# ShengkaiWu/IoU-aware-single-stage-object-detector

Hardware: AMD Instinct MI355X
Metric: images/sec at 1333x800, IoU-aware RetinaNet R-50-FPN (higher is better)
Workload: dtype fp32; 1 GPU; IoU-aware RetinaNet R-50-FPN fp32, batch 8 per GPU, 3x800x1344 (1333x800 padded to /32), random-init weights, whole inference path incl. NMS, device-to-host copy and bbox2result (the reference's simple_test: per-class arrays on the host; batch i's host part runs under batch i+1's device part, the last one inside the timed region); global_batch=8, parallelism=dp1, dets_per_image=100

## Files before the change

include/iouaware.h:

```cpp
#ifndef IOUAWARE_H
#define IOUAWARE_H

#include <stddef.h>
#include <stdint.h>

#ifdef __cplusplus
extern "C" {
#endif

#define IA_MAX_LEVELS 8
#define IA_MAX_ANCHORS 16
#define IA_MAX_NMS_PRE 4096
#define IA_MAX_CANDIDATES 8192
#define IA_MAX_PER_IMG 1024

#define IA_F32 0
#define IA_BF16 1
#define IA_F16 2
#define IA_F64 3

#define IA_LAYOUT_NCHW 0
#define IA_LAYOUT_NHWC 1

#define IA_CLS_SIGMOID 0
// ... 83 lines not shown
                       void *workspace, size_t workspace_bytes, float *dets, int32_t *labels,
                       int32_t *rows, int32_t *num, void *stream);

size_t ia_multiclass_nms_lazy_workspace_bytes(int batch, int R, int C);
int ia_multiclass_nms_lazy(const float *boxes, const float *scores_t, const float *best_score,
                           int batch, int R, int C, float score_thr, float iou_thr,
                           int max_per_img, int candidates, void *workspace,
                           size_t workspace_bytes, float *dets, int32_t *labels, int32_t *rows,
                           int32_t *num, void *stream);

int ia_decode_stage(const ia_head_geom *g, const ia_level_ptrs *p, int batch, int dtype,
                    const float *img_hw, const float *scale_factor, int rescale, void *workspace,
                    size_t workspace_bytes, void *stream);

int ia_get_bboxes_workspace_layout(const ia_head_geom *g, int batch, size_t offsets[8]);

size_t ia_nms_workspace_bytes(int n);
int ia_nms(const float *dets, int n, float iou_thr, int32_t *keep, int32_t *count, void *workspace,
           size_t workspace_bytes, void *stream);

size_t ia_nms_f64_workspace_bytes(int n);
int ia_nms_f64(const double *dets, int n, float iou_thr, int32_t *keep, int32_t *count,
               void *workspace, size_t workspace_bytes, void *stream);

int ia_soft_nms(const float *dets, int n, float iou_thr, int method, float sigma, float min_score,
                float *out_dets, int32_t *out_inds, int32_t *count, void *stream);

typedef struct {
    const uint8_t *src;
    int32_t src_h, src_w, dst_h, dst_w, flip;
} ia_image_desc;
int ia_image_transform(const ia_image_desc *imgs, int batch, const float *mean, const float *std,
                       int to_rgb, int pad_h, int pad_w, int channels_last, float *out,
                       void *stream);

typedef struct {
    int32_t num_levels, batch;
    int32_t H[IA_MAX_LEVELS], W[IA_MAX_LEVELS];
} ia_wino_geom;
typedef struct {
    int32_t c0, n;
    int32_t dst_channels, dst_offset;
    float *dst[IA_MAX_LEVELS];
} ia_wino_seg;
int ia_wino_tiles(const ia_wino_geom *g, int32_t *tiles);
int ia_wino_input_transform(const ia_wino_geom *g, const float *const *x, int channels, int groups,
                            const float *pre_scale, const float *pre_shift, int pre_relu, float *V,
                            void *stream);
int ia_wino_output_transform(const ia_wino_geom *g, const float *M, int channels, int groups,
                             const float *bias, int relu, int nseg, const ia_wino_seg *segs,
                             void *stream);
int ia_wino_mid_transform(const ia_wino_geom *g, const float *M, int channels, int groups_m,
                          const float *bias, int relu, float *V, int groups_v, void *stream);

int ia_wino_grad_output_transform(const ia_wino_geom *g, const float *const *dy, int channels,
                                  float *dM, void *stream);

#define IA_COLSUM_MAX_STRIPS 512
size_t ia_relu_bwd_bias_grad_workspace_bytes(int64_t rows, int n);
int ia_wino_weight_transform(const float *w, int n_in, int n_out, int64_t stride_in,
                             int64_t stride_out, int64_t stride_ky, int64_t stride_kx, int flip,
                             const double *G, float *U, void *stream);
int ia_wino_weight_grad(const float *dU, int n_in, int n_out, const double *G, float *dW,
                        int64_t stride_in, int64_t stride_out, int64_t stride_ky, int64_t stride_kx,
                        void *stream);
int ia_bn_fold_fwd(const float *w, const float *gamma, const float *beta, const float *mean,
                   const float *inv_std, int cout, int K, float *w_out, float *b_out, void *stream);
int ia_bn_fold_bwd(const float *dw_folded, const float *db_folded, const float *w, const float *gamma,
                   const float *mean, const float *inv_std, int cout, int K, float *dw,
                   float *dgamma, float *dbeta, void *stream);
int ia_relu_bwd_bias_grad(const float *dy, const float *y, int64_t rows, int n, float *g, float *db,
                          void *workspace, size_t workspace_bytes, void *stream);

int ia_linear_bias_act(const float *A, const float *W, const float *bias, const float *residual,
                       float *D, int64_t rows, int k, int n, int relu, void *workspace,
                       size_t workspace_bytes, void *stream);
int ia_linear_bias_act_bf16(const void *A, const void *W, const float *bias, const void *residual,
                            void *D, int64_t rows, int k, int n, int relu, void *workspace,
                            size_t workspace_bytes, void *stream);
int ia_batched_gemm(const float *A, const float *W, float *D, int batch, int64_t rows, int k, int n,
                    void *workspace, size_t workspace_bytes, void *stream);
int ia_batched_gemm_stream(const float *A, const float *W, float *D, int batch, int64_t rows, int k,
                           int n, void *stream);

size_t ia_im2col3x3_bytes(int B, int H, int W, int C, int stride, int dtype);
int ia_im2col3x3_nhwc(const void *x, void *col, int B, int H, int W, int C, int stride, int dtype,
                      void *stream);
int ia_conv1x1_strided(const void *x, const void *W_kn, const float *bias, const void *residual,
                       void *D, int B, int H, int W, int k, int n, int stride, int relu, int dtype,
                       void *workspace, size_t workspace_bytes, void *stream);
int ia_col2im3x3_nhwc(const void *dcol, void *dx, int B, int H, int W, int C, int stride, int dtype,
                      void *stream);

int ia_gemm_tuning(int mode);

int ia_gemm_table_add(int64_t m, int64_t n, int64_t k, int flags, int batch, int dtype,
                      int solution_index);
int ia_gemm_table_clear(void);
int ia_gemm_table_dump(int64_t *rows7, int capacity);
int ia_gemm_table_stats(int64_t *hits_misses_stale);
int ia_gemm_library_version(void);

int ia_linear_bias_act_wt(const float *A, const float *W_nk, const float *bias,
                          const float *residual, float *D, int64_t rows, int k, int n, int relu,
                          void *workspace, size_t workspace_bytes, void *stream);
int ia_gemm_tn(const float *G, const float *X, float *D, int batch, int64_t rows, int n, int k,
               void *workspace, size_t workspace_bytes, void *stream);


int ia_focal_loss_fwd(const void *cls, int dtype, const int64_t *labels,
                      const float *label_weights, int B, int A, int C, int HW, float gamma,
                      float alpha, double *loss_sum, void *stream);
int ia_focal_loss_bwd(const void *cls, int dtype, const int64_t *labels,
                      const float *label_weights, int B, int A, int C, int HW, float gamma,
                      float alpha, float gscale, const float *gscale_dev, float *grad_cls,
                      void *stream);

int ia_smooth_l1_fwd(const void *pred, int dtype, const float *target, const float *weight,
                     int B, int A, int HW, float beta, double *loss_sum, void *stream);
int ia_smooth_l1_bwd(const void *pred, int dtype, const float *target, const float *weight,
                     int B, int A, int HW, float beta, float gscale, const float *gscale_dev,
                     float *grad_pred, void *stream);

int ia_focal_loss_balanced_fwd(const void *cls, int dtype, const int64_t *labels,
                               const float *label_weights, const float *anchor_iou, int B, int A,
                               int C, int HW, float gamma, float alpha, float eta,
                               double *loss_sums3, void *stream);
int ia_focal_loss_balanced_bwd(const void *cls, int dtype, const int64_t *labels,
                               const float *label_weights, const float *anchor_iou, int B, int A,
                               int C, int HW, float gamma, float alpha, float eta,
                               const float *normalizer_dev, float gscale, const float *gscale_dev,
                               float *grad_cls, void *stream);
int ia_smooth_l1_balanced_fwd(const void *pred, int dtype, const float *target,
                              const float *weight, const float *anchor_iou, int B, int A, int HW,
                              float beta, float delta, double *loss_sum, void *stream);
int ia_smooth_l1_balanced_bwd(const void *pred, int dtype, const float *target,
                              const float *weight, const float *anchor_iou, int B, int A, int HW,
                              float beta, float delta, float gscale, const float *gscale_dev,
                              float *grad_pred, void *stream);

int ia_iou_bce_fwd(const ia_head_geom *g, int level, const void *bbox_pred, const void *iou_pred,
                   int dtype, const float *bbox_targets, const float *bbox_weights, int B,
                   float *iou_target, double *loss_sum, void *stream);
int ia_iou_bce_bwd(const ia_head_geom *g, int level, const void *bbox_pred, const void *iou_pred,
                   int dtype, const float *bbox_targets, const float *bbox_weights, int B,
                   float gscale, const float *gscale_dev, float *grad_iou_pred,
                   float *grad_bbox_pred, void *stream);

int ia_anchor_targets(const ia_head_geom *g, const float *gt_boxes, const int64_t *gt_labels,
                      const int32_t *num_gt, int batch, int gmax, const int32_t *valid_hw,
                      float pos_iou_thr, float neg_iou_thr, float min_pos_iou, float pos_weight,
                      uint32_t *gt_max_scratch, int64_t *labels, float *label_weights,
                      float *bbox_targets, float *bbox_weights, int32_t *counts, void *stream);

#define IA_MAX_TARGET_BATCH 16
int ia_anchor_targets_ptrs(const ia_head_geom *g, const float *const *gt_boxes,
                           const int64_t *const *gt_labels, const int32_t *num_gt, int batch,
                           const int32_t *valid_hw, float pos_iou_thr, float neg_iou_thr,
                           float min_pos_iou, float pos_weight, uint32_t *gt_max_scratch,
                           int64_t *labels, float *label_weights, float *bbox_targets,
                           float *bbox_weights, int32_t *counts, void *stream);

typedef struct ia_head_targets {
    const int64_t *labels[IA_MAX_LEVELS];
    const float *label_weights[IA_MAX_LEVELS];
    const float *bbox_targets[IA_MAX_LEVELS];
// ... 252 lines not shown
```

iou-aware-single-stage-object-detector_amd/csrc/build.py:

```python
import os
import subprocess
import sys

HERE = os.path.dirname(os.path.abspath(__file__))
SOURCES = ['capi.hip', 'decode.hip', 'select.hip', 'nms.hip', 'loss.hip', 'elementwise.hip', 'assign.hip',
           'softnms.hip', 'preproc.hip', 'wino.hip', 'gemm.hip', 'lazynms.hip', 'headloss.hip', 'gconv.hip',
           'trainops.hip', 'bignms.hip', 'conv3x3_bf16.hip', 'conv3x3_bf16_bwd.hip', 'conv1x1_stream.hip', 'im2col.hip', 'nms64.hip', 'stem.hip',
           'groupnorm.hip', 'pointdecode.hip', 'pointloss.hip', 'gconv_bf16.hip']
HEADERS = ['ia_math.hpp', 'ia_block.hpp', 'ia_internal.hpp', 'ia_loss.hpp', 'ia_headloss.hpp', 'ia_rowmax_dev.hpp', 'ia_gather_dev.hpp', 'ia_nms.hpp', 'ia_conv3.hpp', 'ia_wino.hpp', '../../include/iouaware.h']
OUT = os.path.join(HERE, 'libiouaware_hip.so')
FLAGS = ['--offload-arch=gfx950', '-O3', '-std=c++17', '-fPIC', '-ffp-contract=off',
         '-fhip-fp32-correctly-rounded-divide-sqrt', '-fno-gpu-rdc',
         '-Wall', '-Wno-unused-function']


def _hipcc():
    for c in (os.environ.get('HIPCC'), '/opt/rocm/bin/hipcc', 'hipcc'):
        if c and (os.path.isabs(c) and os.path.exists(c) or not os.path.isabs(c)):
            return c
    return 'hipcc'


def needs_build():
    if not os.path.exists(OUT):
        return True
    t = os.path.getmtime(OUT)
    deps = [os.path.join(HERE, f) for f in SOURCES + HEADERS] + [os.path.abspath(__file__)]
    return any(os.path.getmtime(d) > t for d in deps)


def build(force=False, verbose=False):
    if not force and not needs_build():
        return OUT
    objs = []
    procs = []
    for src in SOURCES:
        obj = os.path.join(HERE, src.replace('.hip', '.o'))
        cmd = [_hipcc()] + FLAGS + ['-c', os.path.join(HERE, src), '-o', obj]
        if verbose:
            print(' '.join(cmd))
        procs.append((src, subprocess.Popen(cmd, stdout=subprocess.PIPE, stderr=subprocess.STDOUT)))
        objs.append(obj)
    for src, pr in procs:
        out, _ = pr.communicate()
        if pr.returncode != 0:
            raise RuntimeError('hipcc failed on %s:\n%s' % (src, out.decode()))
        if verbose and out:
            print(out.decode())
    cmd = [_hipcc(), '--offload-arch=gfx950', '-shared', '-fPIC', '-o', OUT] + objs + [
        '-L/opt/rocm/lib', '-lhipblaslt', '-Wl,-rpath,/opt/rocm/lib']
    subprocess.run(cmd, check=True)
    return OUT


if __name__ == '__main__':
    print(build(force='--force' in sys.argv, verbose=True))
```

iou-aware-single-stage-object-detector_amd/csrc/ia_wino.hpp:

```cpp
#pragma once
#include "ia_internal.hpp"

namespace ia {

struct WinoLevels {
    int32_t L, B;
    int32_t H[IA_MAX_LEVELS], W[IA_MAX_LEVELS], tx[IA_MAX_LEVELS], tpi[IA_MAX_LEVELS];
    int32_t tile_off[IA_MAX_LEVELS + 1];
};

static inline int make_wino_levels(const ia_wino_geom *g, WinoLevels &w)
{
    if (!g || g->num_levels < 1 || g->num_levels > IA_MAX_LEVELS || g->batch < 1) return IA_E_ARG;
    w.L = g->num_levels; w.B = g->batch;
    w.tile_off[0] = 0;
    for (int l = 0; l < IA_MAX_LEVELS; ++l) {
        const bool on = l < g->num_levels;
        if (on && (g->H[l] < 1 || g->W[l] < 1)) return IA_E_ARG;
        w.H[l] = on ? g->H[l] : 0; w.W[l] = on ? g->W[l] : 0;
        w.tx[l] = (w.W[l] + 3) / 4;
        w.tpi[l] = ((w.H[l] + 3) / 4) * w.tx[l];
        const int64_t n = (int64_t)w.tile_off[l] + (int64_t)g->batch * w.tpi[l];
        if (n > 2147483647LL) return IA_E_ARG;
        w.tile_off[l + 1] = (int32_t)n;
    }
    return 0;
}

struct TileRef { int l, b, y0, x0; };

__device__ __forceinline__ int xcd_tile(int bid, int T)
{
    const int per = (T + 7) / 8;
    return (bid & 7) * per + (bid >> 3);
}

__device__ __forceinline__ TileRef locate_tile(const WinoLevels &w, int t, int *Hout = nullptr,
                                               int *Wout = nullptr)
{
    TileRef r;
    int l = 0;
#pragma unroll
    for (int i = 1; i < IA_MAX_LEVELS; ++i) l += (i < w.L && t >= w.tile_off[i]) ? 1 : 0;
    int off = w.tile_off[0], tpi = w.tpi[0], tx = w.tx[0], H = w.H[0], W = w.W[0];
#pragma unroll
    for (int i = 1; i < IA_MAX_LEVELS; ++i) {
        const bool m = l == i;
        off = m ? w.tile_off[i] : off; tpi = m ? w.tpi[i] : tpi; tx = m ? w.tx[i] : tx;
        H = m ? w.H[i] : H; W = m ? w.W[i] : W;
    }
    if (Hout) *Hout = H;
    if (Wout) *Wout = W;
    const int q = t - off;
    r.l = l; r.b = q / tpi;
    const int i = q - r.b * tpi;
    const int ty = i / tx;
    r.y0 = 4 * ty; r.x0 = 4 * (i - ty * tx);
    return r;
}

template <typename P>
__device__ __forceinline__ P opaque(P v)
{
    asm volatile("" : "+s"(v));
    return v;
}
template <bool UNIFORM, typename P>
__device__ __forceinline__ P level_ptr(P const (&tab)[IA_MAX_LEVELS], int l)
{
    if (UNIFORM) return tab[l];
    const char *base = reinterpret_cast<const char *>(tab[0]);
    int64_t d = 0;
#pragma unroll
    for (int i = 1; i < IA_MAX_LEVELS; ++i) {
        const int64_t di = opaque((int64_t)(reinterpret_cast<const char *>(tab[i]) - base));
        d = (l == i) ? di : d;
    }
    return reinterpret_cast<P>(const_cast<char *>(base + d));
}


constexpr int kMaxSeg = 4;

struct WinoSeg {
    int32_t c0, n, Cdst, coff;
    float *dst[IA_MAX_LEVELS];
};

}
```

iou-aware-single-stage-object-detector_amd/csrc/wino.hip:

```cpp
#include <string.h>
#include "ia_internal.hpp"
#include "ia_wino.hpp"

namespace ia {

typedef float f32x4_t __attribute__((ext_vector_type(4)));
__device__ __forceinline__ float4 load_nt(const float *p)
{
    const f32x4_t q = __builtin_nontemporal_load(reinterpret_cast<const f32x4_t *>(p));
    return make_float4(q.x, q.y, q.z, q.w);
}
__device__ __forceinline__ void store_nt(float *p, const float4 &v)
{
    f32x4_t q; q.x = v.x; q.y = v.y; q.z = v.z; q.w = v.w;
    __builtin_nontemporal_store(q, reinterpret_cast<f32x4_t *>(p));
}
__device__ __forceinline__ float4 f4(float v) { return make_float4(v, v, v, v); }
__device__ __forceinline__ float4 operator+(const float4 &a, const float4 &b) { return make_float4(a.x + b.x, a.y + b.y, a.z + b.z, a.w + b.w); }
__device__ __forceinline__ float4 operator-(const float4 &a, const float4 &b) { return make_float4(a.x - b.x, a.y - b.y, a.z - b.z, a.w - b.w); }
__device__ __forceinline__ float4 operator*(float s, const float4 &a) { return make_float4(s * a.x, s * a.y, s * a.z, s * a.w); }

__device__ __forceinline__ void bt6(const float4 (&d)[6], float4 (&o)[6])
{
    o[0] = (4.0f * d[0] - 5.0f * d[2]) + d[4];
    o[1] = (d[3] + d[4]) - 4.0f * (d[1] + d[2]);
    o[2] = 4.0f * (d[1] - d[2]) + (d[4] - d[3]);
    o[3] = 2.0f * (d[3] - d[1]) + (d[4] - d[2]);
    o[4] = 2.0f * (d[1] - d[3]) + (d[4] - d[2]);
    o[5] = (4.0f * d[1] - 5.0f * d[3]) + d[5];
}

__device__ __forceinline__ void at6(const float4 (&m)[6], float4 (&o)[4])
{
    const float4 s12 = m[1] + m[2], d12 = m[1] - m[2], s34 = m[3] + m[4], d34 = m[3] - m[4];
    o[0] = (m[0] + s12) + s34;
    o[1] = d12 + 2.0f * d34;
    o[2] = s12 + 4.0f * s34;
    o[3] = (d12 + 8.0f * d34) + m[5];
}

struct WinoInArgs {
    WinoLevels lv;
    const float *x[IA_MAX_LEVELS];
    float *V;
    const float *pre_scale, *pre_shift;
    int32_t Ctot, Cg, T, pre_relu, tpw;
};

struct LaneMap { int t, c; bool on; };
template <bool PACKED>
__device__ __forceinline__ LaneMap lane_map(int Ctot, int T, int tpw)
{
    LaneMap m;
    const int lane = threadIdx.x;
    if (PACKED) {
        const int q = Ctot >> 2;
        const int sub = lane / q;
        const int tw = xcd_tile(blockIdx.x, (T + tpw - 1) / tpw) * tpw + sub;
        m.t = tw; m.c = (lane - sub * q) * 4;
        m.on = (sub < tpw) && (tw < T);
    } else {
        m.t = __builtin_amdgcn_readfirstlane(xcd_tile(blockIdx.x, T));
        m.c = (blockIdx.y * 64 + lane) * 4;
        m.on = (m.c < Ctot) && (m.t < T);
    }
    return m;
}
static int tiles_per_wave(int channels)
{
    const int q = channels / 4;
    return (q < 64) ? (64 / q) : 1;
}

template <bool PACKED>
__global__ void __launch_bounds__(64) k_wino_in(WinoInArgs a)
{
    const LaneMap lm = lane_map<PACKED>(a.Ctot, a.T, a.tpw);
    if (!lm.on) return;
    const int t = lm.t, c = lm.c;
    int H, W;
    const TileRef r = locate_tile(a.lv, t, &H, &W);
    const float *x = level_ptr<!PACKED>(a.x, r.l) + (size_t)r.b * H * W * a.Ctot + c;
    const bool pre = a.pre_shift != nullptr;
    float4 ps = f4(1.0f), pb = f4(0.0f);
    if (pre) {
        if (a.pre_scale) ps = *reinterpret_cast<const float4 *>(a.pre_scale + c);
        pb = *reinterpret_cast<const float4 *>(a.pre_shift + c);
    }
    float4 d[6][6];
#pragma unroll
    for (int i = 0; i < 6; ++i) {
        const int y = r.y0 - 1 + i;
        const int yc = (y >= 0 && y < H) ? y : 0;
#pragma unroll
        for (int j = 0; j < 6; ++j) {
            const int xx = r.x0 - 1 + j;
            const int xc = (xx >= 0 && xx < W) ? xx : 0;
            d[i][j] = *reinterpret_cast<const float4 *>(x + ((size_t)yc * W + xc) * a.Ctot);
        }
    }
    if (pre) {
        const bool relu = a.pre_relu != 0;
#pragma unroll
        for (int i = 0; i < 6; ++i)
#pragma unroll
            for (int j = 0; j < 6; ++j) {
                float4 v = d[i][j];
                v = make_float4(v.x * ps.x + pb.x, v.y * ps.y + pb.y, v.z * ps.z + pb.z, v.w * ps.w + pb.w);
                const float4 z = make_float4(v.x > 0.f ? v.x : 0.f, v.y > 0.f ? v.y : 0.f,
                                             v.z > 0.f ? v.z : 0.f, v.w > 0.f ? v.w : 0.f);
                d[i][j] = relu ? z : v;
            }
    }
#pragma unroll
    for (int i = 0; i < 6; ++i) {
        const int y = r.y0 - 1 + i;
        const bool yin = (y >= 0) && (y < H);
#pragma unroll
        for (int j = 0; j < 6; ++j) {
            const int xx = r.x0 - 1 + j;
            const bool in = yin && (xx >= 0) && (xx < W);
// ... 416 lines not shown
```

iou-aware-single-stage-object-detector_amd/iouaware/_lib.py:

```python
import ctypes as C
import os

IA_MAX_LEVELS = 8
IA_MAX_ANCHORS = 16
IA_MAX_NMS_PRE = 4096
IA_MAX_CANDIDATES = 8192
IA_MAX_PER_IMG = 1024
IA_F32, IA_BF16, IA_F16, IA_F64 = 0, 1, 2, 3
IA_LAYOUT_NCHW, IA_LAYOUT_NHWC = 0, 1
IA_CLS_SIGMOID, IA_CLS_SOFTMAX = 0, 1
IA_CLS_SIGMOID_NOIOU, IA_CLS_SOFTMAX_NOIOU = 2, 3
IA_LOSS_SLOTS = 64
IA_MAX_TARGET_BATCH = 16
IA_GN_CHUNK = 256

_CSRC = os.path.join(os.path.dirname(os.path.abspath(__file__)), '..', 'csrc')
SO_PATH = os.path.abspath(os.path.join(_CSRC, 'libiouaware_hip.so'))


class HeadGeom(C.Structure):
    _fields_ = [('num_levels', C.c_int32), ('num_anchors', C.c_int32),
                ('num_classes', C.c_int32), ('nms_pre', C.c_int32),
                ('H', C.c_int32 * IA_MAX_LEVELS), ('W', C.c_int32 * IA_MAX_LEVELS),
                ('stride', C.c_int32 * IA_MAX_LEVELS),
# ... 49 lines not shown


class ImageDesc(C.Structure):
    _fields_ = [('src', C.c_void_p), ('src_h', C.c_int32), ('src_w', C.c_int32),
                ('dst_h', C.c_int32), ('dst_w', C.c_int32), ('flip', C.c_int32)]


class WinoGeom(C.Structure):
    _fields_ = [('num_levels', C.c_int32), ('batch', C.c_int32),
                ('H', C.c_int32 * IA_MAX_LEVELS), ('W', C.c_int32 * IA_MAX_LEVELS)]


class Conv3x3Desc(C.Structure):
    _fields_ = [('num_levels', C.c_int32), ('batch', C.c_int32), ('groups', C.c_int32),
                ('cin', C.c_int32), ('cout', C.c_int32), ('x_stride', C.c_int32), ('y_stride', C.c_int32),
                ('H', C.c_int32 * IA_MAX_LEVELS), ('W', C.c_int32 * IA_MAX_LEVELS),
                ('x', (C.c_void_p * IA_MAX_LEVELS) * 2), ('y', (C.c_void_p * IA_MAX_LEVELS) * 2)]


class WinoSeg(C.Structure):
    _fields_ = [('c0', C.c_int32), ('n', C.c_int32), ('dst_channels', C.c_int32),
                ('dst_offset', C.c_int32), ('dst', C.c_void_p * IA_MAX_LEVELS)]


_vp, _i, _f, _sz, _i64 = C.c_void_p, C.c_int, C.c_float, C.c_size_t, C.c_int64
_G, _P = C.POINTER(HeadGeom), C.POINTER(LevelPtrs)
_PG, _WG = C.POINTER(PointHeadGeom), C.POINTER(WinoGeom)
_PP, _PT, _PC = C.POINTER(PointLevelPtrs), C.POINTER(PointTargets), C.POINTER(PointLossCfg)

SIGNATURES = {
    'ia_version': (C.c_char_p, []),
    'ia_geom_sizes': (_i, [_G, C.POINTER(C.c_int32), C.POINTER(C.c_int32), C.POINTER(C.c_int32)]),
    'ia_decode_fuse_rowmax': (_i, [_G, _P, _i, _i, _vp, _vp]),
    'ia_select_topk_workspace_bytes': (_sz, [_G, _i]),
    'ia_select_topk': (_i, [_G, _vp, _i, _vp, _vp, _sz, _vp]),
    'ia_decode_fuse_rowmax_grouped': (_i, [_G, _P, _i, _i, _vp, _vp, _sz, _vp]),
    'ia_select_topk_grouped': (_i, [_G, _vp, _i, _vp, _vp, _sz, _vp]),
    'ia_decode_stage': (_i, [_G, _P, _i, _i, _vp, _vp, _i, _vp, _sz, _vp]),
    'ia_get_bboxes_status_offset': (_sz, [_G, _i]),
    'ia_debug_fused_spin_limit': (_i, [_i64]),
    'ia_profile_stage_events': (_i, [_vp, _vp]),
    'ia_gather_decode': (_i, [_G, _P, _i, _i, _vp, _vp, _vp, _i, _vp, _vp, _vp, _vp]),
    'ia_multiclass_nms_workspace_bytes': (_sz, [_i, _i, _i]),
    'ia_multiclass_nms': (_i, [_vp, _vp, _vp, _i, _i, _i, _f, _f, _i, _vp, _sz, _vp, _vp, _vp,
                               _vp, _vp, _vp, _vp]),
    'ia_multiclass_soft_nms_workspace_bytes': (_sz, [_i, _i, _i]),
    'ia_multiclass_soft_nms': (_i, [_vp, _vp, _i, _i, _i, _f, _f, _i, _f, _f, _i, _vp, _sz, _vp, _vp,
                                    _vp, _vp, _vp, _vp, _vp]),
    'ia_soft_nms': (_i, [_vp, _i, _f, _i, _f, _f, _vp, _vp, _vp, _vp]),
    'ia_get_bboxes_workspace_bytes': (_sz, [_G, _i]),
    'ia_get_bboxes': (_i, [_G, _P, _i, _i, _vp, _vp, _i, _f, _f, _i, _vp, _sz, _vp, _vp, _vp,
                           _vp, _vp]),
    'ia_multiclass_nms_lazy_workspace_bytes': (_sz, [_i, _i, _i]),
    'ia_multiclass_nms_lazy': (_i, [_vp, _vp, _vp, _i, _i, _i, _f, _f, _i, _i, _vp, _sz, _vp, _vp, _vp,
                                    _vp, _vp]),
    'ia_get_bboxes_lazy': (_i, [_G, _P, _i, _i, _vp, _vp, _i, _f, _f, _i, _i, _vp, _sz, _vp, _vp, _vp,
                                _vp, _vp]),
    'ia_get_bboxes_workspace_layout': (_i, [_G, _i, C.POINTER(_sz * 8)]),
    'ia_nms_workspace_bytes': (_sz, [_i]),
    'ia_nms': (_i, [_vp, _i, _f, _vp, _vp, _vp, _sz, _vp]),
    'ia_nms_f64_workspace_bytes': (_sz, [_i]),
    'ia_nms_f64': (_i, [_vp, _i, _f, _vp, _vp, _vp, _sz, _vp]),
    'ia_image_transform': (_i, [C.POINTER(ImageDesc), _i, C.POINTER(C.c_float), C.POINTER(C.c_float),
                                _i, _i, _i, _i, _vp, _vp]),
    'ia_wino_tiles': (_i, [C.POINTER(WinoGeom), C.POINTER(C.c_int32)]),
    'ia_wino_input_transform': (_i, [C.POINTER(WinoGeom), C.POINTER(C.c_void_p), _i, _i, _vp, _vp, _i,
                                     _vp, _vp]),
    'ia_wino_grad_output_transform': (_i, [C.POINTER(WinoGeom), C.POINTER(C.c_void_p), _i, _vp, _vp]),
    'ia_wino_weight_transform': (_i, [_vp, _i, _i, C.c_int64, C.c_int64, C.c_int64, C.c_int64, _i,
                                      C.POINTER(C.c_double), _vp, _vp]),
    'ia_wino_weight_grad': (_i, [_vp, _i, _i, C.POINTER(C.c_double), _vp, C.c_int64, C.c_int64,
                                 C.c_int64, C.c_int64, _vp]),
    'ia_bn_fold_fwd': (_i, [_vp, _vp, _vp, _vp, _vp, _i, _i, _vp, _vp, _vp]),
    'ia_bn_fold_bwd': (_i, [_vp, _vp, _vp, _vp, _vp, _vp, _i, _i, _vp, _vp, _vp, _vp]),
    'ia_relu_bwd_bias_grad_workspace_bytes': (C.c_size_t, [C.c_int64, _i]),
    'ia_relu_bwd_bias_grad': (_i, [_vp, _vp, C.c_int64, _i, _vp, _vp, _vp, C.c_size_t, _vp]),
    'ia_wino_output_transform': (_i, [C.POINTER(WinoGeom), _vp, _i, _i, _vp, _i, _i,
                                      C.POINTER(WinoSeg), _vp]),
    'ia_wino_mid_transform': (_i, [C.POINTER(WinoGeom), _vp, _i, _i, _vp, _i, _vp, _i, _vp]),
    'ia_linear_bias_act': (_i, [_vp, _vp, _vp, _vp, _vp, _i64, _i, _i, _i, _vp, _sz, _vp]),
    'ia_linear_bias_act_bf16': (_i, [_vp, _vp, _vp, _vp, _vp, _i64, _i, _i, _i, _vp, _sz, _vp]),
    'ia_batched_gemm': (_i, [_vp, _vp, _vp, _i, _i64, _i, _i, _vp, _sz, _vp]),
    'ia_batched_gemm_stream': (_i, [_vp, _vp, _vp, _i, _i64, _i, _i, _vp]),
    'ia_linear_bias_act_wt': (_i, [_vp, _vp, _vp, _vp, _vp, _i64, _i, _i, _i, _vp, _sz, _vp]),
    'ia_gemm_tuning': (_i, [_i]),
    'ia_im2col3x3_bytes': (_sz, [_i, _i, _i, _i, _i, _i]),
    'ia_im2col3x3_nhwc': (_i, [_vp, _vp, _i, _i, _i, _i, _i, _i, _vp]),
    'ia_col2im3x3_nhwc': (_i, [_vp, _vp, _i, _i, _i, _i, _i, _i, _vp]),
    'ia_conv1x1_strided': (_i, [_vp, _vp, _vp, _vp, _vp, _i, _i, _i, _i, _i, _i, _i, _i, _vp, _sz, _vp]),
    'ia_gemm_table_add': (_i, [_i64, _i64, _i64, _i, _i, _i, _i]),
    'ia_gemm_table_clear': (_i, []),
    'ia_gemm_table_dump': (_i, [_vp, _i]),
    'ia_gemm_table_stats': (_i, [_vp]),
    'ia_gemm_library_version': (_i, []),
    'ia_gemm_tn': (_i, [_vp, _vp, _vp, _i, _i64, _i, _i, _vp, _sz, _vp]),
    'ia_focal_loss_fwd': (_i, [_vp, _i, _vp, _vp, _i, _i, _i, _i, _f, _f, _vp, _vp]),
    'ia_focal_loss_bwd': (_i, [_vp, _i, _vp, _vp, _i, _i, _i, _i, _f, _f, _f, _vp, _vp, _vp]),
    'ia_smooth_l1_fwd': (_i, [_vp, _i, _vp, _vp, _i, _i, _i, _f, _vp, _vp]),
    'ia_smooth_l1_bwd': (_i, [_vp, _i, _vp, _vp, _i, _i, _i, _f, _f, _vp, _vp, _vp]),
    'ia_focal_loss_balanced_fwd': (_i, [_vp, _i, _vp, _vp, _vp, _i, _i, _i, _i, _f, _f, _f, _vp, _vp]),
    'ia_focal_loss_balanced_bwd': (_i, [_vp, _i, _vp, _vp, _vp, _i, _i, _i, _i, _f, _f, _f, _vp, _f,
                                        _vp, _vp, _vp]),
    'ia_smooth_l1_balanced_fwd': (_i, [_vp, _i, _vp, _vp, _vp, _i, _i, _i, _f, _f, _vp, _vp]),
    'ia_smooth_l1_balanced_bwd': (_i, [_vp, _i, _vp, _vp, _vp, _i, _i, _i, _f, _f, _f, _vp, _vp,
                                       _vp]),
    'ia_iou_bce_fwd': (_i, [_G, _i, _vp, _vp, _i, _vp, _vp, _i, _vp, _vp, _vp]),
    'ia_iou_bce_bwd': (_i, [_G, _i, _vp, _vp, _i, _vp, _vp, _i, _f, _vp, _vp, _vp, _vp]),
    'ia_anchor_targets': (_i, [_G, _vp, _vp, _vp, _i, _i, _vp, _f, _f, _f, _f, _vp, _vp, _vp, _vp,
                               _vp, _vp, _vp]),
    'ia_anchor_targets_ptrs': (_i, [_G, C.POINTER(C.c_void_p), C.POINTER(C.c_void_p),
                                    C.POINTER(C.c_int32), _i, C.POINTER(C.c_int32), _f, _f, _f, _f,
                                    _vp, _vp, _vp, _vp, _vp, _vp, _vp]),
    'ia_head_loss_workspace_bytes': (_sz, [_G, _i]),
    'ia_head_loss_fwd': (_i, [_G, _P, _i, _i, C.POINTER(HeadTargets), C.POINTER(HeadLossCfg), _vp,
                              _sz, _vp, _vp]),
    'ia_head_loss_bwd': (_i, [_G, _P, _i, _i, C.POINTER(HeadTargets), C.POINTER(HeadLossCfg), _vp,
                              _vp, _vp, _P, _vp]),
    'ia_head_loss_fwd_nhwc': (_i, [_G, _P, C.POINTER(LevelPixStrides), _i, C.POINTER(HeadTargets),
                                   C.POINTER(HeadLossCfg), _vp, _sz, _vp, _vp]),
    'ia_head_loss_bwd_nhwc': (_i, [_G, _P, C.POINTER(LevelPixStrides), _i, C.POINTER(HeadTargets),
                                   C.POINTER(HeadLossCfg), _vp, _vp, _P, C.POINTER(LevelPixStrides),
                                   _vp]),
    'ia_grouped_conv3x3_pack': (_i, [_vp, _vp, _i, _i, _vp]),
    'ia_grouped_conv3x3_nhwc': (_i, [_vp, _vp, _vp, _vp, _i, _i, _i, _i, _i, _i, _i, _vp]),
    'ia_grouped_conv3x3_packed_bytes_bf16': (C.c_size_t, [_i, _i]),
    'ia_grouped_conv3x3_pack_bf16': (_i, [_vp, _vp, _i, _i, _vp]),
    'ia_grouped_conv3x3_bf16_nhwc': (_i, [_vp, _vp, _vp, _vp, _i, _i, _i, _i, _i, _i, _i, _vp]),
    'ia_sigmoid_focal_loss_fwd': (_i, [_vp, _vp, _i, _i, _f, _f, _vp, _vp]),
    'ia_sigmoid_focal_loss_bwd': (_i, [_vp, _vp, _vp, _i, _i, _f, _f, _vp, _vp]),
    'ia_sigmoid_focal_loss_fwd_dt': (_i, [_vp, _i, _vp, _i, _i, _f, _f, _vp, _vp]),
    'ia_sigmoid_focal_loss_bwd_dt': (_i, [_vp, _i, _vp, _vp, _i, _i, _f, _f, _vp, _vp]),
    'ia_channel_affine_act': (_i, [_vp, _i, _vp, _vp, _vp, _vp, _vp, _i, _i, _i, _i64, _vp]),
    'ia_channel_affine_act_nhwc': (_i, [_vp, _i, _vp, _vp, _vp, _vp, _vp, _i, _i64, _i, _vp]),
    'ia_nhwc_to_nchw': (_i, [_vp, _vp, _i, _i, _i, _i64, _vp]),
    'ia_upsample2x_add_nhwc': (_i, [_vp, _vp, _i, _i, _i, _i, _i, _i, _vp]),
    'ia_conv1x1_stream': (_i, [_vp, _vp, _vp, _vp, _vp, C.c_int64, _i, _i, _i, _vp]),
    'ia_stem_conv7x7s2': (_i, [_vp, _vp, _vp, _i, _i, _i, _vp]),
    'ia_stem_conv7x7s2_bf16': (_i, [_vp, _vp, _vp, _i, _i, _i, _vp]),
    'ia_conv1x1_wide': (_i, [_vp, _vp, _vp, _vp, _vp, C.c_int64, _i, _i, _i, _vp]),
    'ia_conv1x1_chain': (_i, [_vp, _vp, _vp, _vp, _vp, _vp, _vp, _vp, _i64, _i, _i, _i, _vp]),
    'ia_conv3x3_bf16_packed_bytes': (C.c_size_t, [_i, _i, _i]),
    'ia_conv3x3_bf16_pack': (_i, [_vp, _i, _i, _i, _vp, _vp]),
    'ia_conv3x3_bf16_levels': (_i, [_vp, _vp, _vp, _i, _vp]),
    'ia_conv3x3_bf16_wgrad_workspace_bytes': (C.c_size_t, [_vp]),
    'ia_conv3x3_bf16_wgrad_plan': (_i, [_vp, C.POINTER(C.c_int32), C.POINTER(C.c_int32), C.POINTER(C.c_int32)]),
    'ia_conv3x3_bf16_wgrad_levels': (_i, [_vp, _vp, _vp, C.c_size_t, _vp]),
    'ia_conv3x3_bf16_pack_f32': (_i, [_vp, _i, _i, _i, _i, _vp, _vp]),
    'ia_relu_bwd_bias_grad_bf16_workspace_bytes': (C.c_size_t, [C.c_int64, _i]),
    'ia_relu_bwd_bias_grad_bf16': (_i, [_vp, C.c_int64, _vp, C.c_int64, C.c_int64, _i, _vp, C.c_int64, _vp,
                                        _vp, C.c_size_t, _vp]),
    'ia_upsample2x_add_nhwc_dt': (_i, [_vp, _vp, _i, _i, _i, _i, _i, _i, _i, _vp]),
    'ia_affine_relu_maxpool_nhwc_dt': (_i, [_vp, _i, _vp, _vp, _i, _i, _i, _i, _vp, _vp]),
    'ia_affine_relu_maxpool_nhwc': (_i, [_vp, _vp, _vp, _i, _i, _i, _i, _vp, _vp]),
    'ia_groupnorm_workspace_bytes': (_sz, [_WG, _i, _i]),
    'ia_groupnorm_stats': (_i, [_WG, C.POINTER(C.c_void_p), _i, _i, _vp, _sz, _vp]),
    'ia_groupnorm_apply': (_i, [_WG, C.POINTER(C.c_void_p), _i, _i, _vp, _vp, _f, _i, _vp, _sz, _vp]),
    'ia_groupnorm_workspace_bytes_dt': (_sz, [_WG, _i, _i, _i]),
    'ia_groupnorm_stats_dt': (_i, [_WG, C.POINTER(C.c_void_p), _i, _i, _i, _vp, _sz, _vp]),
    'ia_groupnorm_apply_dt': (_i, [_WG, C.POINTER(C.c_void_p), _i, _i, _i, _vp, _vp, _f, _i, _vp, _sz,
                                   _vp]),
    'ia_groupnorm_saved_bytes': (_sz, [_WG, _i, _i]),
    'ia_groupnorm_apply_to': (_i, [_WG, C.POINTER(C.c_void_p), C.POINTER(C.c_void_p), _i, _i, _vp, _vp, _f,
                                   _i, _vp, _sz, _vp, _sz, _vp]),
    'ia_groupnorm_bwd_workspace_bytes': (_sz, [_WG, _i, _i]),
    'ia_groupnorm_bwd_reduce': (_i, [_WG, C.POINTER(C.c_void_p), C.POINTER(C.c_void_p), _i, _i, _vp, _vp, _i,
                                     _vp, _sz, _vp, _sz, _vp]),
# ... 72 lines not shown
```

iou-aware-single-stage-object-detector_amd/iouaware/winograd.py:

```python
import collections
import ctypes as C

import numpy as np
import torch

from . import _lib
from .ops import _ptr, _stream, stream_id

_G = np.array([[1 / 4, 0, 0], [-1 / 6, -1 / 6, -1 / 6], [-1 / 6, 1 / 6, -1 / 6],
               [1 / 24, 1 / 12, 1 / 6], [1 / 24, -1 / 12, 1 / 6], [0, 0, 1]], dtype=np.float64)


_G_DEV = {}


def transform_weight(w):
    if w.dim() != 4 or w.shape[2] != 3 or w.shape[3] != 3:
        raise ValueError('Winograd F(4,3) needs a 3x3 kernel, got %s' % (tuple(w.shape),))
    g = w.detach().to(torch.float64)
    G = _G_DEV.get(g.device)
    if G is None:
        G = _G_DEV[g.device] = torch.from_numpy(_G).to(g.device)
    u = torch.einsum('ik,ockl,jl->ijco', G, g, G)
    return u.reshape(36, g.shape[1], g.shape[0]).to(torch.float32).contiguous()
# ... 25 lines not shown
    n = 1
    for d in shape:
        n *= int(d)
    key = (device, stream_id(), name)
    b = _SCRATCH.get(key)
    if b is None or b.numel() < n:
        b = _SCRATCH[key] = torch.empty(n, dtype=torch.float32, device=device)
    return b[:n].view(*shape)


_PLAN_ENTRIES = 4


def _plan_for(plans, key, make):
    plan = plans.get(key)
    if plan is None:
        while len(plans) >= _PLAN_ENTRIES:
            plans.popitem(last=False)
        plan = plans[key] = make()
    else:
        plans.move_to_end(key)
    return plan


class _Plan(object):

    def __init__(self, sizes, batch, device):
        self.sizes, self.batch = list(sizes), batch
        self.geom = _wino_geom(sizes, batch)
        self.T = _wino_tiles(self.geom)
        self.device = device
        self._bufs = {}

    def buf(self, name, shape):
        return _scratch(self.device, name, shape)

    def acts(self, name, channels):
        key = ('acts', name, channels)
        a = self._bufs.get(key)
        if a is None:
            a = [torch.empty((self.batch, channels, h, w), dtype=torch.float32, device=self.device,
                             memory_format=torch.channels_last) for (h, w) in self.sizes]
            self._bufs[key] = a
        return a


TIMING = None


def _timed(kind, nbytes, launch):
    if TIMING is None:
        return launch()
    e0, e1 = torch.cuda.Event(enable_timing=True), torch.cuda.Event(enable_timing=True)
    e0.record()
    launch()
    e1.record()
    TIMING.append((kind, e0, e1, nbytes))


def input_transform(plan, xs, groups, out, pre=None):
    ptrs = (C.c_void_p * len(xs))(*[x.data_ptr() for x in xs])
    ps, pb, pr = pre if pre is not None else (None, None, False)
    ch = int(xs[0].shape[1])
    _timed('in', plan.T * ch * 4 * (16 + 36), lambda: _lib.check(
        _lib.lib().ia_wino_input_transform(C.byref(plan.geom), ptrs, ch, int(groups), _ptr(ps),
                                           _ptr(pb), int(bool(pr)), _ptr(out), _stream()),
        'ia_wino_input_transform'))
    return out


def output_transform(plan, m, channels, groups, bias, relu, segments):
    segs = (_lib.WinoSeg * len(segments))()
    for k, (c0, n, dst, off) in enumerate(segments):
        segs[k].c0, segs[k].n = int(c0), int(n)
        segs[k].dst_channels, segs[k].dst_offset = int(dst[0].shape[1]), int(off)
        for l, t in enumerate(dst):
            segs[k].dst[l] = t.data_ptr()
    _timed('out', plan.T * int(channels) * 4 * (36 + 16), lambda: _lib.check(
        _lib.lib().ia_wino_output_transform(C.byref(plan.geom), _ptr(m), int(channels), int(groups),
                                            _ptr(bias), int(bool(relu)), len(segments), segs,
                                            _stream()), 'ia_wino_output_transform'))


MID_CHANNELS = 32


def mid_transform(plan, m, channels, groups_m, bias, relu, out, groups_v):
    _timed('mid', plan.T * int(channels) * 4 * (36 + 36), lambda: _lib.check(
        _lib.lib().ia_wino_mid_transform(C.byref(plan.geom), _ptr(m), int(channels), int(groups_m),
                                         _ptr(bias), int(bool(relu)), _ptr(out), int(groups_v),
                                         _stream()), 'ia_wino_mid_transform'))
    return out


_LT_WS_BYTES = 128 << 20


STREAM_BMM = True
_STREAM_BMM_SHAPES = ((64, 64),)


def batched_gemm(v, u, out):
    from . import ops
    ops._ensure_gemm_table()
    batch, rows, k = v.shape
    n = u.shape[2]
    if not (v.is_contiguous() and u.is_contiguous() and out.is_contiguous()):
        raise ValueError('batched_gemm needs contiguous stacks')
    if STREAM_BMM and (k, n) in _STREAM_BMM_SHAPES and rows >= 4096 and v.dtype == torch.float32:
        _lib.check(_lib.lib().ia_batched_gemm_stream(_ptr(v), _ptr(u), _ptr(out), int(batch), int(rows),
                                                     int(k), int(n), _stream()), 'ia_batched_gemm_stream')
        return out
    ws = _scratch(v.device, 'lt_ws', (_LT_WS_BYTES // 4,))
    _lib.check(_lib.lib().ia_batched_gemm(_ptr(v), _ptr(u), _ptr(out), int(batch), int(rows), int(k),
                                          int(n), _ptr(ws), _LT_WS_BYTES, _stream()),
               'ia_batched_gemm')
    return out


class WinogradConv3x3(object):

    def __init__(self, weight, bias, relu=False):
        self.u = transform_weight(weight)
        self.bias = None if bias is None else bias.detach().to(torch.float32).contiguous()
        self.relu = relu
        self.cin, self.cout = self.u.shape[1], self.u.shape[2]
        if self.cout % 4:
            raise ValueError('output channels must be a multiple of 4')
        self._plans = collections.OrderedDict()

    def usable(self, x):
        return _usable(x) and x.shape[1] == self.cin \
            and not (torch.is_grad_enabled() and x.requires_grad)

    def __call__(self, x, pre=None):
        key = (x.shape[0], tuple(x.shape[-2:]), x.device, stream_id())
        plan = _plan_for(self._plans, key, lambda: _Plan([tuple(x.shape[-2:])], x.shape[0], x.device))
        v = input_transform(plan, [x], 1, plan.buf('v', (36, plan.T, self.cin)), pre)
        m = batched_gemm(v, self.u, plan.buf('m', (36, plan.T, self.cout)))
        y = torch.empty((x.shape[0], self.cout) + tuple(x.shape[-2:]), dtype=torch.float32,
                        device=x.device, memory_format=torch.channels_last)
        output_transform(plan, m, self.cout, 1, self.bias, self.relu, [(0, self.cout, [y], 0)])
        return y


def plain_3x3(conv):
    return (tuple(conv.kernel_size) == (3, 3) and tuple(conv.stride) == (1, 1)
            and tuple(conv.padding) == (1, 1) and tuple(conv.dilation) == (1, 1) and conv.groups == 1)


def _pair(a, b, F, granule):
    na, nb = a.out_channels, (0 if b is None else b.out_channels)
    n_pad = (na + nb + granule - 1) // granule * granule
    dev = a.weight.device
    u = torch.zeros((36, F, n_pad), dtype=torch.float32, device=dev)
    u[:, :, :na] = transform_weight(a.weight)
    bias = torch.zeros(n_pad, dtype=torch.float32, device=dev)
    bias[:na] = a.bias.detach().float()
    if b is not None:
        u[:, :, na:na + nb] = transform_weight(b.weight)
        bias[na:na + nb] = b.bias.detach().float()
    return u.contiguous(), bias.contiguous(), na, nb


class _WinogradTowers(object):

    FUSE_MID = True
    mid_bias = None

    def __init__(self, head):
        convs_c, convs_r = list(head.cls_convs), list(head.reg_convs)
        self.n_layers = len(convs_c)
        F = head.feat_channels
        if head.in_channels % 4 or F % 4:
            raise ValueError('channel counts must be multiples of 4')
        self.F, self.cin = F, head.in_channels
        self.u0 = torch.cat([transform_weight(convs_c[0].conv.weight),
                             transform_weight(convs_r[0].conv.weight)], dim=2).contiguous()
        self.u = [torch.cat([transform_weight(convs_c[i].conv.weight),
                             transform_weight(convs_r[i].conv.weight)], dim=0).contiguous()
                  for i in range(1, self.n_layers)]
        self._plans = collections.OrderedDict()

    def usable(self, feats):
        return all(_usable(x) and x.shape[1] == self.cin for x in feats) \
            and not torch.is_grad_enabled()

    def _towers(self, feats):
        B, dev = feats[0].shape[0], feats[0].device
        sizes = [tuple(x.shape[-2:]) for x in feats]
        key = (B, tuple(sizes), dev, stream_id())
        plan = _plan_for(self._plans, key, lambda: _Plan(sizes, B, dev))
        T, F = plan.T, self.F
        v = input_transform(plan, feats, 1, plan.buf('v', (36, T, self.cin)))
        m = batched_gemm(v, self.u0, plan.buf('m', (36, T, 2 * F)))
        new = lambda c: [torch.empty((B, c, h, w), dtype=torch.float32, device=dev,
                                     memory_format=torch.channels_last) for (h, w) in sizes]
        if self.FUSE_MID and self.mid_bias is not None and F % MID_CHANNELS == 0:
            groups = 1
            for i, u in enumerate(self.u):
                v = mid_transform(plan, m, 2 * F, groups, self.mid_bias[i], True,
                                  plan.buf('v', (72, T, F)), 2)
                m = batched_gemm(v, u, plan.buf('m', (72, T, F)))
                groups = 2
            v = mid_transform(plan, m, 2 * F, groups, self.mid_bias[self.n_layers - 1], True,
                              plan.buf('v', (72, T, F)), 2)
            return plan, v, new
        acts = plan.acts('a', 2 * F)
        self._layer_out(plan, m, 1, 0, acts)
        for i, u in enumerate(self.u):
            v = input_transform(plan, acts, 2, plan.buf('v', (72, T, F)))
            m = batched_gemm(v, u, plan.buf('m', (72, T, F)))
            nxt = plan.acts('b' if acts is plan.acts('a', 2 * F) else 'a', 2 * F)
            self._layer_out(plan, m, 2, i + 1, nxt)
            acts = nxt
        v = input_transform(plan, acts, 2, plan.buf('v', (72, T, F)))
        return plan, v, new

    @staticmethod
    def _out_conv(plan, v, name, u, bias, segments):
        n = u.shape[2]
        m = batched_gemm(v, u, plan.buf(name, (36, plan.T, n)))
        output_transform(plan, m, n, 1, bias, False, segments)

# ... 90 lines not shown
```

Baseline: 412.6 img/s.

## Fuse Winograd batched GEMM with output transform for 64x64 convs

Adds a kernel that computes all 36 Winograd-domain products for a block of 16 tiles with MFMA, keeps them in registers, and applies the output transform, bias and ReLU directly to the NHWC output. This removes writing and re-reading the 36xTx64 intermediate product tensor for 64-channel 3x3 convs large enough to use the streaming GEMM path. The cost is 144 accumulator VGPRs per lane and a fixed workgroup/LDS mapping limited to 64x64 channels and at most 4 levels.

```diff
diff --git a/include/iouaware.h b/include/iouaware.h
--- a/include/iouaware.h
+++ b/include/iouaware.h
@@ -189,6 +189,8 @@
                     void *workspace, size_t workspace_bytes, void *stream);
 int ia_batched_gemm_stream(const float *A, const float *W, float *D, int batch, int64_t rows, int k,
                            int n, void *stream);
+int ia_wino_prod_out(const ia_wino_geom *g, const float *V, const float *U, int k, int n,
+                     const float *bias, int relu, float *const *dst, void *stream);
 
 size_t ia_im2col3x3_bytes(int B, int H, int W, int C, int stride, int dtype);
 int ia_im2col3x3_nhwc(const void *x, void *col, int B, int H, int W, int C, int stride, int dtype,
diff --git a/iou-aware-single-stage-object-detector_amd/csrc/build.py b/iou-aware-single-stage-object-detector_amd/csrc/build.py
--- a/iou-aware-single-stage-object-detector_amd/csrc/build.py
+++ b/iou-aware-single-stage-object-detector_amd/csrc/build.py
@@ -6,7 +6,7 @@
 SOURCES = ['capi.hip', 'decode.hip', 'select.hip', 'nms.hip', 'loss.hip', 'elementwise.hip', 'assign.hip',
            'softnms.hip', 'preproc.hip', 'wino.hip', 'gemm.hip', 'lazynms.hip', 'headloss.hip', 'gconv.hip',
            'trainops.hip', 'bignms.hip', 'conv3x3_bf16.hip', 'conv3x3_bf16_bwd.hip', 'conv1x1_stream.hip', 'im2col.hip', 'nms64.hip', 'stem.hip',
-           'groupnorm.hip', 'pointdecode.hip', 'pointloss.hip', 'gconv_bf16.hip']
+           'groupnorm.hip', 'pointdecode.hip', 'pointloss.hip', 'gconv_bf16.hip', 'wino_prod.hip']
 HEADERS = ['ia_math.hpp', 'ia_block.hpp', 'ia_internal.hpp', 'ia_loss.hpp', 'ia_headloss.hpp', 'ia_rowmax_dev.hpp', 'ia_gather_dev.hpp', 'ia_nms.hpp', 'ia_conv3.hpp', 'ia_wino.hpp', '../../include/iouaware.h']
 OUT = os.path.join(HERE, 'libiouaware_hip.so')
 FLAGS = ['--offload-arch=gfx950', '-O3', '-std=c++17', '-fPIC', '-ffp-contract=off',
diff --git a/iou-aware-single-stage-object-detector_amd/csrc/ia_wino.hpp b/iou-aware-single-stage-object-detector_amd/csrc/ia_wino.hpp
--- a/iou-aware-single-stage-object-detector_amd/csrc/ia_wino.hpp
+++ b/iou-aware-single-stage-object-detector_amd/csrc/ia_wino.hpp
@@ -79,6 +79,19 @@
     return reinterpret_cast<P>(const_cast<char *>(base + d));
 }
 
+__device__ __forceinline__ float4 f4(float v) { return make_float4(v, v, v, v); }
+__device__ __forceinline__ float4 operator+(const float4 &a, const float4 &b) { return make_float4(a.x + b.x, a.y + b.y, a.z + b.z, a.w + b.w); }
+__device__ __forceinline__ float4 operator-(const float4 &a, const float4 &b) { return make_float4(a.x - b.x, a.y - b.y, a.z - b.z, a.w - b.w); }
+__device__ __forceinline__ float4 operator*(float s, const float4 &a) { return make_float4(s * a.x, s * a.y, s * a.z, s * a.w); }
+
+__device__ __forceinline__ void at6(const float4 (&m)[6], float4 (&o)[4])
+{
+    const float4 s12 = m[1] + m[2], d12 = m[1] - m[2], s34 = m[3] + m[4], d34 = m[3] - m[4];
+    o[0] = (m[0] + s12) + s34;
+    o[1] = d12 + 2.0f * d34;
+    o[2] = s12 + 4.0f * s34;
+    o[3] = (d12 + 8.0f * d34) + m[5];
+}
 
 constexpr int kMaxSeg = 4;
 
diff --git a/iou-aware-single-stage-object-detector_amd/csrc/wino.hip b/iou-aware-single-stage-object-detector_amd/csrc/wino.hip
--- a/iou-aware-single-stage-object-detector_amd/csrc/wino.hip
+++ b/iou-aware-single-stage-object-detector_amd/csrc/wino.hip
@@ -15,10 +15,6 @@
     f32x4_t q; q.x = v.x; q.y = v.y; q.z = v.z; q.w = v.w;
     __builtin_nontemporal_store(q, reinterpret_cast<f32x4_t *>(p));
 }
-__device__ __forceinline__ float4 f4(float v) { return make_float4(v, v, v, v); }
-__device__ __forceinline__ float4 operator+(const float4 &a, const float4 &b) { return make_float4(a.x + b.x, a.y + b.y, a.z + b.z, a.w + b.w); }
-__device__ __forceinline__ float4 operator-(const float4 &a, const float4 &b) { return make_float4(a.x - b.x, a.y - b.y, a.z - b.z, a.w - b.w); }
-__device__ __forceinline__ float4 operator*(float s, const float4 &a) { return make_float4(s * a.x, s * a.y, s * a.z, s * a.w); }
 
 __device__ __forceinline__ void bt6(const float4 (&d)[6], float4 (&o)[6])
 {
@@ -28,15 +24,6 @@
     o[3] = 2.0f * (d[3] - d[1]) + (d[4] - d[2]);
     o[4] = 2.0f * (d[1] - d[3]) + (d[4] - d[2]);
     o[5] = (4.0f * d[1] - 5.0f * d[3]) + d[5];
-}
-
-__device__ __forceinline__ void at6(const float4 (&m)[6], float4 (&o)[4])
-{
-    const float4 s12 = m[1] + m[2], d12 = m[1] - m[2], s34 = m[3] + m[4], d34 = m[3] - m[4];
-    o[0] = (m[0] + s12) + s34;
-    o[1] = d12 + 2.0f * d34;
-    o[2] = s12 + 4.0f * s34;
-    o[3] = (d12 + 8.0f * d34) + m[5];
 }
 
 struct WinoInArgs {
diff --git a/iou-aware-single-stage-object-detector_amd/csrc/wino_prod.hip b/iou-aware-single-stage-object-detector_amd/csrc/wino_prod.hip
--- /dev/null
+++ b/iou-aware-single-stage-object-detector_amd/csrc/wino_prod.hip
@@ -0,0 +1,184 @@
+#include "ia_internal.hpp"
+#include "ia_wino.hpp"
+
+namespace ia {
+
+typedef __attribute__((ext_vector_type(4))) float f32x4;
+
+constexpr int kProdLevels = 4;
+
+struct WinoProdArgs {
+    WinoLevels lv;
+    const float *V, *U, *bias;
+    float *dst[kProdLevels];
+    int32_t T, nblocks, nslots, relu;
+};
+
+constexpr int kProdThreads = 512;
+constexpr int kProdWaves = kProdThreads / 64;
+
+template <int K, int N>
+__global__ void __launch_bounds__(kProdThreads) k_wino_prod_out(WinoProdArgs a)
+{
+    static_assert(K == 64 && N == 64, "the workgroup -> (channel block, tile group) map and the LDS budget are for 64 x 64");
+    constexpr int J = K / 16, PL = K * 16;
+    __shared__ __attribute__((aligned(16))) float s_u[36 * PL];
+    const int tid = threadIdx.x, lane = tid & 63;
+    const int bid = blockIdx.x;
+    const int nbk = (bid >> 3) & 3;
+    const int grp = (bid & 7) + 8 * (bid >> 5), ngrp = a.nslots / kProdWaves;
+    if (grp >= a.nblocks) return;
+    {
+        constexpr int NU = 36 * K * 4 / kProdThreads;
+        static_assert(NU * kProdThreads == 36 * K * 4, "whole passes");
+        const float *u = a.U + nbk * 16;
+        float4 w[NU];
+#pragma unroll
+        for (int it = 0; it < NU; ++it) {
+            const int i = tid + it * kProdThreads;
+            const int n4 = i & 3, k = (i >> 2) & (K - 1), pl = i / (4 * K);
+            w[it] = *reinterpret_cast<const float4 *>(u + ((size_t)pl * K + k) * N + 4 * n4);
+        }
+#pragma unroll
+        for (int it = 0; it < NU; ++it) {
+            const int i = tid + it * kProdThreads;
+            const int n4 = i & 3, k = (i >> 2) & (K - 1), pl = i / (4 * K);
+            float *d = s_u + pl * PL + (k >> 4) * 256 + (((k >> 2) & 3) * 16 + 4 * n4) * 4 + (k & 3);
+            d[0] = w[it].x; d[4] = w[it].y; d[8] = w[it].z; d[12] = w[it].w;
+        }
+    }
+    __syncthreads();
+
+    const int p_in = lane & 15, q = lane >> 4;
+    int blk = __builtin_amdgcn_readfirstlane(tid >> 6) * ngrp + grp;
+    if (blk >= a.nblocks) return;
+    const int cb = nbk * 16 + 4 * q;
+    const size_t kstride = (size_t)a.T * K;
+    const int tlast = a.T - 1;
+    auto vrow = [&](int b) {
+        const int t0 = b * 16 + p_in;
+        const int tc = t0 < tlast ? t0 : tlast;
+        return a.V + ((size_t)tc * K + 4 * q);
+    };
+
+    f32x4 xv[3][J];
+    const float *vr = vrow(blk);
+#pragma unroll
+    for (int j = 0; j < J; ++j) {
+        xv[0][j] = *reinterpret_cast<const f32x4 *>(vr + 16 * j);
+    }
+    for (;;) {
+        const int nxt = blk + a.nslots;
+        const bool more = nxt < a.nblocks;
+#pragma unroll
+        for (int j = 0; j < J; ++j) xv[1][j] = *reinterpret_cast<const f32x4 *>(vr + kstride + 16 * j);
+        f32x4 uf[2][J];
+#pragma unroll
+        for (int j = 0; j < J; ++j) uf[0][j] = *reinterpret_cast<const f32x4 *>(s_u + j * 256 + lane * 4);
+        f32x4 acc[36];
+#pragma unroll
+        for (int pl = 0; pl < 36; ++pl) {
+            if (pl + 2 == 36) vr = vrow(more ? nxt : blk);
+            if (pl + 2 <= 36) {
+                const float *src = vr + (size_t)((pl + 2) % 36) * kstride;
+#pragma unroll
+                for (int j = 0; j < J; ++j) xv[(pl + 2) % 3][j] = *reinterpret_cast<const f32x4 *>(src + 16 * j);
+            }
+            if (pl + 1 < 36) {
+                int ln = lane;
+                asm volatile("" : "+v"(ln));
+#pragma unroll
+                for (int j = 0; j < J; ++j)
+                    uf[(pl + 1) & 1][j] = *reinterpret_cast<const f32x4 *>(s_u + (pl + 1) * PL + j * 256 + ln * 4);
+            }
+            f32x4 c = f32x4{0.0f, 0.0f, 0.0f, 0.0f};
+#pragma unroll
+            for (int j = 0; j < J; ++j)
+#pragma unroll
+                for (int cc = 0; cc < 4; ++cc)
+                    c = __builtin_amdgcn_mfma_f32_16x16x4f32(uf[pl & 1][j][cc], xv[pl % 3][j][cc], c, 0, 0, 0);
+            acc[pl] = c;
+            __builtin_amdgcn_sched_barrier(0);
+        }
+
+        const int t0 = blk * 16 + p_in;
+        if (t0 < a.T) {
+            int H, W;
+            WinoLevels lv = a.lv;
+            const int L = opaque(lv.L);
+            lv.L = L < kProdLevels ? L : kProdLevels;
+            const TileRef r = locate_tile(lv, t0, &H, &W);
+            int cbo = cb;
+            asm volatile("" : "+v"(cbo));
+            int64_t doff = 0;
+#pragma unroll
+            for (int i = 1; i < kProdLevels; ++i) {
+                const int64_t di = opaque((int64_t)(reinterpret_cast<const char *>(a.dst[i]) - reinterpret_cast<const char *>(a.dst[0])));
+                doff = (r.l == i) ? di : doff;
+            }
+            float *dst = reinterpret_cast<float *>(reinterpret_cast<char *>(a.dst[0]) + doff) + cbo;
+            float4 bz = f4(0.0f);
+            if (a.bias) bz = *reinterpret_cast<const float4 *>(a.bias + cbo);
+            float4 s[4][6];
+#pragma unroll
+            for (int j = 0; j < 6; ++j) {
+                float4 col[6], o[4];
+#pragma unroll
+                for (int i = 0; i < 6; ++i) {
+                    const f32x4 m = acc[i * 6 + j];
+                    col[i] = make_float4(m.x, m.y, m.z, m.w);
+                }
+                at6(col, o);
+#pragma unroll
+                for (int i = 0; i < 4; ++i) s[i][j] = o[i];
+                __builtin_amdgcn_sched_barrier(0);
+            }
+#pragma unroll
+            for (int i = 0; i < 4; ++i) {
+                float4 o[4];
+                at6(s[i], o);
+                const int y = r.y0 + i;
+#pragma unroll
+                for (int j = 0; j < 4; ++j) {
+                    const int xx = r.x0 + j;
+                    if (y >= H || xx >= W) continue;
+                    float4 v = o[j] + bz;
+                    if (a.relu) v = make_float4(v.x > 0.f ? v.x : 0.f, v.y > 0.f ? v.y : 0.f,
+                                                v.z > 0.f ? v.z : 0.f, v.w > 0.f ? v.w : 0.f);
+                    const size_t pix = ((size_t)r.b * H + y) * W + xx;
+                    *reinterpret_cast<float4 *>(dst + pix * N) = v;
+                }
+            }
+        }
+        if (!more) break;
+        blk = nxt;
+    }
+}
+
+}
+
+extern "C" int ia_wino_prod_out(const ia_wino_geom *g, const float *V, const float *U, int k, int n,
+                                const float *bias, int relu, float *const *dst, void *stream)
+{
+    ia::WinoProdArgs a;
+    int rc = ia::make_wino_levels(g, a.lv);
+    if (rc) return rc;
+    if (!V || !U || !dst || a.lv.L > ia::kProdLevels) return IA_E_ARG;
+    if (k != 64 || n != 64) return IA_E_ARG;
+    if (((uintptr_t)V & 15u) || ((uintptr_t)U & 15u) || ((uintptr_t)bias & 15u)) return IA_E_ARG;
+    for (int l = 0; l < ia::kProdLevels; ++l) {
+        a.dst[l] = (l < a.lv.L) ? dst[l] : nullptr;
+        if (l < a.lv.L && (!dst[l] || ((uintptr_t)dst[l] & 15u))) return IA_E_ARG;
+    }
+    a.T = a.lv.tile_off[a.lv.L];
+    if (a.T < 1 || a.T > 2147483647 - 16) return IA_E_ARG;
+    a.V = V; a.U = U; a.bias = bias; a.relu = relu ? 1 : 0;
+    a.nblocks = (a.T + 15) / 16;
+    int groups = (a.nblocks + ia::kProdWaves - 1) / ia::kProdWaves;
+    groups = (groups + 7) / 8 * 8;
+    if (groups > 64) groups = 64;
+    a.nslots = groups * ia::kProdWaves;
+    hipLaunchKernelGGL((ia::k_wino_prod_out<64, 64>), dim3((unsigned)(4 * groups)), dim3(ia::kProdThreads), 0,
+                       (hipStream_t)stream, a);
+    return ia::hip_status(hipGetLastError());
+}
diff --git a/iou-aware-single-stage-object-detector_amd/iouaware/_lib.py b/iou-aware-single-stage-object-detector_amd/iouaware/_lib.py
--- a/iou-aware-single-stage-object-detector_amd/iouaware/_lib.py
+++ b/iou-aware-single-stage-object-detector_amd/iouaware/_lib.py
@@ -155,6 +155,7 @@
     'ia_linear_bias_act_bf16': (_i, [_vp, _vp, _vp, _vp, _vp, _i64, _i, _i, _i, _vp, _sz, _vp]),
     'ia_batched_gemm': (_i, [_vp, _vp, _vp, _i, _i64, _i, _i, _vp, _sz, _vp]),
     'ia_batched_gemm_stream': (_i, [_vp, _vp, _vp, _i, _i64, _i, _i, _vp]),
+    'ia_wino_prod_out': (_i, [C.POINTER(WinoGeom), _vp, _vp, _i, _i, _vp, _i, C.POINTER(C.c_void_p), _vp]),
     'ia_linear_bias_act_wt': (_i, [_vp, _vp, _vp, _vp, _vp, _i64, _i, _i, _i, _vp, _sz, _vp]),
     'ia_gemm_tuning': (_i, [_i]),
     'ia_im2col3x3_bytes': (_sz, [_i, _i, _i, _i, _i, _i]),
diff --git a/iou-aware-single-stage-object-detector_amd/iouaware/winograd.py b/iou-aware-single-stage-object-detector_amd/iouaware/winograd.py
--- a/iou-aware-single-stage-object-detector_amd/iouaware/winograd.py
+++ b/iou-aware-single-stage-object-detector_amd/iouaware/winograd.py
@@ -131,6 +131,14 @@
                                             _stream()), 'ia_wino_output_transform'))
 
 
+def prod_out_transform(plan, v, u, bias, relu, dst):
+    ptrs = (C.c_void_p * len(dst))(*[t.data_ptr() for t in dst])
+    k, n = int(u.shape[1]), int(u.shape[2])
+    _timed('prod_out', plan.T * n * 4 * (36 + 16), lambda: _lib.check(
+        _lib.lib().ia_wino_prod_out(C.byref(plan.geom), _ptr(v), _ptr(u), k, n, _ptr(bias),
+                                    int(bool(relu)), ptrs, _stream()), 'ia_wino_prod_out'))
+
+
 MID_CHANNELS = 32
 
 
@@ -147,6 +155,12 @@
 
 STREAM_BMM = True
 _STREAM_BMM_SHAPES = ((64, 64),)
+_STREAM_BMM_ROWS = 4096
+
+
+def _streamed(v, k, n):
+    return (STREAM_BMM and (k, n) in _STREAM_BMM_SHAPES and v.shape[1] >= _STREAM_BMM_ROWS
+            and v.dtype == torch.float32)
 
 
 def batched_gemm(v, u, out):
@@ -156,7 +170,7 @@
     n = u.shape[2]
     if not (v.is_contiguous() and u.is_contiguous() and out.is_contiguous()):
         raise ValueError('batched_gemm needs contiguous stacks')
-    if STREAM_BMM and (k, n) in _STREAM_BMM_SHAPES and rows >= 4096 and v.dtype == torch.float32:
+    if _streamed(v, k, n):
         _lib.check(_lib.lib().ia_batched_gemm_stream(_ptr(v), _ptr(u), _ptr(out), int(batch), int(rows),
                                                      int(k), int(n), _stream()), 'ia_batched_gemm_stream')
         return out
@@ -169,6 +183,8 @@
 
 class WinogradConv3x3(object):
 
+    FUSE_PROD_OUT = True
+
     def __init__(self, weight, bias, relu=False):
         self.u = transform_weight(weight)
         self.bias = None if bias is None else bias.detach().to(torch.float32).contiguous()
@@ -186,9 +202,12 @@
         key = (x.shape[0], tuple(x.shape[-2:]), x.device, stream_id())
         plan = _plan_for(self._plans, key, lambda: _Plan([tuple(x.shape[-2:])], x.shape[0], x.device))
         v = input_transform(plan, [x], 1, plan.buf('v', (36, plan.T, self.cin)), pre)
-        m = batched_gemm(v, self.u, plan.buf('m', (36, plan.T, self.cout)))
         y = torch.empty((x.shape[0], self.cout) + tuple(x.shape[-2:]), dtype=torch.float32,
                         device=x.device, memory_format=torch.channels_last)
+        if self.FUSE_PROD_OUT and _streamed(v, self.cin, self.cout):
+            prod_out_transform(plan, v, self.u, self.bias, self.relu, [y])
+            return y
+        m = batched_gemm(v, self.u, plan.buf('m', (36, plan.T, self.cout)))
         output_transform(plan, m, self.cout, 1, self.bias, self.relu, [(0, self.cout, [y], 0)])
         return y
 
```

New measurement: 416.9 img/s (median of 6 runs). 1.0% higher.
